# Godotcoffee/AlignGraph2

Measured on AMD Instinct MI355X. Metric: aligned-read-bases/sec through PAGraph build+traverse, higher is better.
Workload: dtype u32

## Files before the change

### aligngraph2_amd/csrc/hip/k1_extract.hip

```cpp
#include "pag_device.hpp"

namespace pagdev {

constexpr int TILE = 1024;
constexpr int CHUNK = 1024;

template <int MAXS>
struct WaveLds {
    uint32_t kept[64];
    uint32_t rank[64];
    uint32_t scode[MAXS];
    uint32_t scnt[MAXS];
    uint32_t srun[MAXS];
    uint32_t st[MAXS];
};
constexpr int MAXS_SPACED = 352;

__device__ __forceinline__ uint32_t load_cols16(const uint32_t *__restrict__ diff, uint64_t diff_off, uint32_t n_cols,
                                                bool back, uint32_t j0, uint32_t *n_lane) {
    if (j0 >= n_cols) {
        *n_lane = 0;
        return 0;
    }
    uint32_t n = n_cols - j0;
    if (n > 16) n = 16;
    *n_lane = n;
    if (!back) return diff[diff_off + (j0 >> 4)];
    int64_t s_lo = (int64_t)n_cols - 16 - (int64_t)j0;
    uint32_t w32;
    if (s_lo >= 0) {
        uint64_t w = diff_off + ((uint64_t)s_lo >> 4);
        uint32_t sh = ((uint32_t)s_lo & 15u) * 2u;
        uint32_t lo = diff[w];
        w32 = lo >> sh;
        if (sh) w32 |= diff[w + 1] << (32 - sh);
    } else {
        uint32_t m = (uint32_t)(-s_lo);
        w32 = diff[diff_off] << (2 * m);
    }
    return rev2(w32);
}

__device__ __forceinline__ void col_masks(uint32_t bits, uint32_t n_lane, uint32_t *emitb, uint32_t *radvb) {
    uint32_t valid = n_lane >= 16 ? 0x55555555u : (((1u << (2 * n_lane)) - 1u) & 0x55555555u);
    uint32_t qd = bits & 0x55555555u, rd = (bits >> 1) & 0x55555555u;
    *emitb = ~(qd & ~rd) & valid;
    *radvb = ~(rd & ~qd) & valid;
}

__global__ __launch_bounds__(64) void colidx_kernel(const pag_aln *__restrict__ aln, uint64_t n_aln,
                                                    const uint32_t *__restrict__ diff,
                                                    const uint64_t *__restrict__ colidx_off, uint2 *__restrict__ colidx) {
    uint64_t ai = blockIdx.x;
    if (ai >= n_aln) return;
    pag_aln al = aln[ai];
    if (!(al.flags & PAG_ALN_ELIGIBLE) || al.query == PAG_NONE) return;
    bool back = (al.flags & PAG_ALN_WALK_BACK) != 0;
    uint32_t n_chunks = (al.n_cols + CHUNK - 1) / CHUNK;
    uint32_t e = 0, r = 0;
    uint64_t base = colidx_off[ai];
    for (uint32_t c = 0; c < n_chunks; ++c) {
        if (lane_id() == 0) colidx[base + c] = make_uint2(e, r);
        uint32_t n_lane, eb, rb;
        uint32_t bits = load_cols16(diff, al.diff_off, al.n_cols, back, c * CHUNK + lane_id() * 16, &n_lane);
        col_masks(bits, n_lane, &eb, &rb);
        e += wave_sum(__popc(eb));
        r += wave_sum(__popc(rb));
    }
}

int launch_colidx(const pag_aln *aln, uint64_t n_aln, const uint32_t *diff, const uint64_t *colidx_off, uint2 *colidx,
                  hipStream_t s) {
    if (n_aln == 0) return PAG_OK;
    colidx_kernel<<<dim3((unsigned)n_aln), dim3(64), 0, s>>>(aln, n_aln, diff, colidx_off, colidx);
    PAG_HIP_TRY(hipGetLastError());
    return PAG_OK;
}

template <typename F>
__device__ __forceinline__ void walk_alignment(const pag_aln &al, const uint32_t *__restrict__ diff,
                                               const uint2 *__restrict__ cidx, uint32_t lo, uint32_t hi, F f) {
    uint32_t q_end = al.q_start + al.n_valid;
    uint32_t a = lo > al.q_start ? lo : al.q_start;
    uint32_t b = hi < q_end ? hi : q_end;
    if (a >= b) return;
    uint32_t e0 = a - al.q_start, e1 = b - al.q_start;
    bool back = (al.flags & PAG_ALN_WALK_BACK) != 0;
    uint32_t n_chunks = (al.n_cols + CHUNK - 1) / CHUNK;
    uint32_t c_lo = 0, c_hi = n_chunks;
    while (c_hi - c_lo > 1) {
        uint32_t mid = (c_lo + c_hi) >> 1;
        if (cidx[mid].x <= e0) c_lo = mid;
        else c_hi = mid;
    }
    for (uint32_t c = c_lo; c < n_chunks; ++c) {
        uint2 pre = cidx[c];
        if (pre.x >= e1) break;
        uint32_t n_lane, eb, rb;
        uint32_t bits = load_cols16(diff, al.diff_off, al.n_cols, back, c * CHUNK + lane_id() * 16, &n_lane);
        col_masks(bits, n_lane, &eb, &rb);
        uint32_t tot;
        uint32_t eex = wave_excl_sum(__popc(eb), &tot) + pre.x;
        uint32_t rex = wave_excl_sum(__popc(rb), &tot) + pre.y;
        uint32_t m = eb;
        while (m) {
            uint32_t bit = __ffs(m) - 1;
            m &= m - 1;
            uint32_t below = (1u << bit) - 1u;
            uint32_t ord = eex + __popc(eb & below);
            if (ord >= e0 && ord < e1) f(al.q_start + ord, al.t_start + rex + __popc(rb & below));
        }
    }
}

__device__ __forceinline__ uint32_t even_bits16(uint32_t x) {
    x &= 0x55555555u;
    x = (x | (x >> 1)) & 0x33333333u;
    x = (x | (x >> 2)) & 0x0F0F0F0Fu;
    x = (x | (x >> 4)) & 0x00FF00FFu;
    return (x | (x >> 8)) & 0xFFFFu;
}
__device__ __forceinline__ uint32_t nth_set_bit16(uint32_t x, uint32_t n) {
    uint32_t pos = 0, c = __popc(x & 0xFFu);
    if (n >= c) n -= c, pos = 8u, x >>= 8;
    c = __popc(x & 0xFu);
    if (n >= c) n -= c, pos += 4u, x >>= 4;
    c = __popc(x & 0x3u);
    if (n >= c) n -= c, pos += 2u, x >>= 2;
    return pos + (n >= (x & 1u) ? 1u : 0u);
}
template <typename G>
__device__ __forceinline__ void walk_kept(const pag_aln &al, const uint32_t *__restrict__ diff, const uint2 *__restrict__ cidx, uint32_t lo,
                                          uint32_t hi, const uint32_t (&kept)[64], const uint32_t (&rank)[64], G g) {
    const uint32_t q_end = al.q_start + al.n_valid;
    const uint32_t a = lo > al.q_start ? lo : al.q_start;
    const uint32_t b = hi < q_end ? hi : q_end;
    if (a >= b) return;
    const uint32_t e0 = a - al.q_start, e1 = b - al.q_start;
    const bool back = (al.flags & PAG_ALN_WALK_BACK) != 0;
    const uint32_t n_chunks = (al.n_cols + CHUNK - 1) / CHUNK;
    uint32_t c_lo = 0, c_hi = n_chunks;
    while (c_hi - c_lo > 1) {
        const uint32_t mid = (c_lo + c_hi) >> 1;
        if (cidx[mid].x <= e0) c_lo = mid;
        else c_hi = mid;
    }
    for (uint32_t c = c_lo; c < n_chunks; ++c) {
        const uint2 pre = cidx[c];
        if (pre.x >= e1) break;
        uint32_t n_lane, eb, rb;
        const uint32_t bits = load_cols16(diff, al.diff_off, al.n_cols, back, c * CHUNK + lane_id() * 16, &n_lane);
        col_masks(bits, n_lane, &eb, &rb);
        const uint32_t ne = __popc(eb);
        uint32_t tot;
        const uint32_t eex = wave_excl_sum(ne, &tot) + pre.x;
        const uint32_t rex = wave_excl_sum(__popc(rb), &tot) + pre.y;
        const uint32_t o_lo = eex > e0 ? eex : e0, o_hi = eex + ne < e1 ? eex + ne : e1;
        if (o_lo >= o_hi) continue;
        const uint32_t d_lo = al.q_start + o_lo - lo, n = o_hi - o_lo;
        const uint32_t w = d_lo >> 4, sh = d_lo & 15u;
        const bool two = sh + n > 16u;
        const uint32_t k0 = kept[w] & 0xFFFFu, k1 = two ? kept[w + 1] & 0xFFFFu : 0u;
        uint32_t km = ((k0 | (k1 << 16)) >> sh) & ((1u << n) - 1u);
        if (!km) continue;
        const uint32_t e16 = even_bits16(eb), r16 = even_bits16(rb);
        const uint32_t r0 = rank[w], r1 = two ? rank[w + 1] : 0u;
        while (km) {
            const uint32_t i = (uint32_t)__ffs((int)km) - 1u;
            km &= km - 1u;
            const uint32_t col = nth_set_bit16(e16, o_lo + i - eex);
            const uint32_t t = al.t_start + rex + __popc(r16 & ((1u << col) - 1u));
            const uint32_t d = d_lo + i;
            const bool first = (d >> 4) == w;
            g((first ? r0 : r1) + __popc((first ? k0 : k1) & ((1u << (d & 15u)) - 1u)), t);
        }
    }
}

__device__ __forceinline__ void lane_codes(const uint32_t *__restrict__ words, uint32_t strand, uint32_t len, uint32_t k,
                                           uint32_t kmask, uint32_t p0, uint32_t n_mine, uint32_t (&code)[16]) {
    uint64_t W = 0;
    uint32_t sh0 = 0;
    if (n_mine) {
        if (strand == 0) {
            uint32_t w0 = p0 >> 4;
            W = (uint64_t)words[w0] | ((uint64_t)words[w0 + 1] << 32);
        } else {
            int64_t a0 = (int64_t)len - (int64_t)k - (int64_t)p0 - 15;
            uint32_t a1 = a0 > 0 ? (uint32_t)a0 : 0u;
            uint32_t w = a1 >> 4, sh = (a1 & 15u) * 2u;
            uint64_t lo64 = (uint64_t)words[w] | ((uint64_t)words[w + 1] << 32);
            W = lo64 >> sh;
            if (sh) W |= (uint64_t)words[w + 2] << (64 - sh);
            sh0 = (uint32_t)((a0 - (int64_t)a1) * 2);
        }
    }
    if (strand == 0) {
        fwd_codes16(W, k, kmask, code);
        return;
    }
#pragma unroll
    for (int j = 0; j < 16; ++j) {
        const uint32_t shj = (uint32_t)(2 * (15 - j)) + sh0;
        const uint32_t x = (uint32_t)(W >> (shj & 63u)) & kmask;
        code[j] = (~x) & kmask;
    }
}

struct LaneWindow {
    uint64_t x = 0;
    uint32_t s0 = 0;
    __device__ __forceinline__ uint32_t code(uint32_t strand, uint32_t kmask, uint32_t j) const {
        if (strand == 0) return (uint32_t)(x >> (s0 - 2u * j)) & kmask;
        return ~(uint32_t)(x >> ((2u * (15u - j) + s0) & 63u)) & kmask;
    }
};
__device__ __forceinline__ LaneWindow lane_window(const uint32_t *__restrict__ words, uint32_t strand, uint32_t len, uint32_t k, uint32_t p0,
                                                  uint32_t n_mine) {
    LaneWindow L;
    if (!n_mine) return L;
    if (strand == 0) {
        const uint32_t w0 = p0 >> 4;
        const uint32_t lo = words[w0], hi = words[w0 + 1];
        L.x = ((uint64_t)rev2(lo) << 32) | (uint64_t)rev2(hi);
        L.s0 = 2u * (32u - k);
    } else {
        const int64_t a0 = (int64_t)len - (int64_t)k - (int64_t)p0 - 15;
        const uint32_t a1 = a0 > 0 ? (uint32_t)a0 : 0u;
        const uint32_t w = a1 >> 4, sh = (a1 & 15u) * 2u;
        const uint64_t lo64 = (uint64_t)words[w] | ((uint64_t)words[w + 1] << 32);
        L.x = lo64 >> sh;
        if (sh) L.x |= (uint64_t)words[w + 2] << (64 - sh);
        L.s0 = (uint32_t)((a0 - (int64_t)a1) * 2);
    }
    return L;
}

constexpr uint32_t SOLID_SLICES = 8;
__global__ __launch_bounds__(64) void solid_mask_kernel(ExtractArgs A, const pag_aln *__restrict__ aln2,
                                                        const uint64_t *__restrict__ qoff2, uint16_t *__restrict__ mask) {
    const uint32_t job = blockIdx.x / SOLID_SLICES, slice = blockIdx.x % SOLID_SLICES;
    const uint32_t lane = lane_id();
    const uint32_t r = A.emit_order[job >> 1];
    const uint32_t strand = job & 1u;
    const uint32_t len = A.read_len[r];
    const uint32_t k = A.k;
    if (len < k) return;
    const uint32_t kmask = k >= 16 ? 0xFFFFFFFFu : ((1u << (2 * k)) - 1u);
    const uint32_t slice_shift = 2 * k - 3;
    const uint32_t *__restrict__ words = (const uint32_t *)(A.packed + A.read_off[r]);
    const uint32_t n_pos = len - k + 1;
    uint32_t lo = 0xFFFFFFFFu, hi = 0;
    for (int db = 0; db < 2; ++db) {
        const pag_aln *al = db == 0 ? A.aln : aln2;
        const uint64_t *qo = db == 0 ? A.query_off : qoff2;
        for (uint64_t ai = qo[r]; ai < qo[r + 1]; ++ai) {
            pag_aln a = al[ai];
            if (!(a.flags & PAG_ALN_ELIGIBLE) || a.q_start == PAG_NONE || a.n_valid == 0) continue;
            if (((a.flags & PAG_ALN_REV_STRAND) ? 1u : 0u) != strand) continue;
            lo = a.q_start < lo ? a.q_start : lo;
            hi = a.q_start + a.n_valid > hi ? a.q_start + a.n_valid : hi;
        }
    }
    if (hi > n_pos) hi = n_pos;
    if (lo >= hi) return;
    uint16_t *m = mask + (uint64_t)slice * A.solid_mask_stride + 2ull * (A.read_off[r] >> 2) + strand;
    for (uint32_t t0 = lo & ~(uint32_t)(TILE - 1); t0 < hi; t0 += TILE) {
        const uint32_t p0 = t0 + lane * 16;
        const uint32_t n_mine = p0 >= n_pos ? 0u : (n_pos - p0 > 16 ? 16u : n_pos - p0);
        if (p0 + 16 <= lo || p0 >= hi || n_mine == 0) continue;
        uint32_t code[16];
        lane_codes(words, strand, len, k, kmask, p0, n_mine, code);
        uint32_t bits = 0;
#pragma unroll
        for (int j = 0; j < 16; ++j)
            if ((uint32_t)j < n_mine && (code[j] >> slice_shift) == slice) bits |= ((A.solid_bits[code[j] >> 5] >> (code[j] & 31u)) & 1u) << j;
        m[2ull * (p0 >> 4)] = (uint16_t)bits;
    }
}

int launch_solid_mask(const ExtractArgs &a, const pag_aln *aln2, const uint64_t *qoff2, uint16_t *mask, hipStream_t s) {
    if (a.n_reads == 0) return PAG_OK;
    solid_mask_kernel<<<dim3(SOLID_SLICES * 2u * a.n_reads), dim3(64), 0, s>>>(a, aln2, qoff2, mask);
    PAG_HIP_TRY(hipGetLastError());
    return PAG_OK;
}
uint32_t solid_mask_slices() { return SOLID_SLICES; }

__device__ __forceinline__ uint32_t tab_get(uint32_t tab, uint32_t s) { return (tab >> (4 * s)) & 15u; }
__device__ __forceinline__ uint32_t byte_compose(uint32_t first, uint32_t then) { return __builtin_amdgcn_perm(then, then, first); }
__device__ __forceinline__ uint32_t byte_get(uint32_t tab, uint32_t s) { return (tab >> (8 * s)) & 255u; }
__device__ __forceinline__ uint32_t tab_compose(uint32_t first, uint32_t then, uint32_t S) {
    uint32_t out = 0;
    for (uint32_t s = 0; s <= S; ++s) out |= tab_get(then, tab_get(first, s)) << (4 * s);
    return out;
}

template <bool EMIT, int MAXS>
__global__ __launch_bounds__(64) void extract_kernel(ExtractArgs A) {
    __shared__ WaveLds<MAXS> L;
    const uint32_t job = A.exec_perm ? A.exec_perm[blockIdx.x] : blockIdx.x;
    const uint32_t lane = lane_id();
    const uint32_t r = A.emit_order[job >> 1];
    const uint32_t strand = job & 1u;
    const uint32_t len = A.read_len[r];
    const uint32_t k = A.k;
    const uint32_t S = A.outer;
    const uint64_t a_lo = A.query_off[r], a_hi = A.query_off[r + 1];
    const uint32_t kmask = k >= 16 ? 0xFFFFFFFFu : ((1u << (2 * k)) - 1u);
    const uint32_t *__restrict__ words = (const uint32_t *)(A.packed + A.read_off[r]);

    auto for_active = [&](auto body) {
        int done = 0;
        for (uint64_t ai = a_lo; ai < a_hi; ++ai) {
            if (A.topk >= 0 && done >= A.topk) break;
            pag_aln al = A.aln[ai];
            if (!(al.flags & PAG_ALN_ELIGIBLE)) continue;
            if (A.cov_ok && !A.cov_ok[ai]) continue;
            ++done;
            if (((al.flags & PAG_ALN_REV_STRAND) ? 1u : 0u) != strand) continue;
            if (al.q_start == PAG_NONE || al.n_valid == 0) continue;
            body(al, ai);
        }
    };

    uint32_t job_samples = 0;
    uint64_t job_tuples = 0;
    bool any = false;
    if (len >= k) for_active([&](const pag_aln &, uint64_t) { any = true; });
    if (!any) {
        if (!EMIT && lane == 0) {
            A.job_samples[A.job_base + job] = 0;
            A.job_tuples[A.job_base + job] = 0;
        }
        return;
    }
    const uint32_t n_pos = len - k + 1;
    bool fast_counts = false;
    if (EMIT) {
        uint32_t n_act = 0;
        bool any_multi = false;
        for_active([&](const pag_aln &al, uint64_t) {
            ++n_act;
            any_multi = any_multi || (A.pass == 0 && A.ctgs[al.target].multi != 0);
        });
        fast_counts = !any_multi && n_act <= 15u;
    }
    const uint64_t tuple_base = EMIT ? A.tuple_off[A.job_base + job] : 0;
    const uint64_t edge_base = EMIT ? A.edge_off[A.job_base + job] : 0;

    uint32_t state = S;
    uint32_t byte_t0 = 0, byte_t1 = 0;
    for (uint32_t st = 0; st < 4u; ++st) {
        byte_t0 |= (st + 1u > S ? S : st + 1u) << (8u * st);
        byte_t1 |= (st + 1u >= S ? 0u : st + 1u) << (8u * st);
    }
    bool carry_valid = false;
    uint32_t carry_pos = 0, carry_code = 0;

    for (uint32_t t0 = 0; t0 < n_pos; t0 += TILE) {
        const uint32_t p0 = t0 + lane * 16;
        const uint32_t t_hi = t0 + TILE < n_pos ? t0 + TILE : n_pos;

        uint32_t ne = 0;
        for_active([&](const pag_aln &al, uint64_t) {
            uint32_t lo = al.q_start > p0 ? al.q_start : p0;
            uint32_t hi = al.q_start + al.n_valid;
            if (hi > p0 + 16) hi = p0 + 16;
            if (hi > n_pos) hi = n_pos;
            if (lo < hi) ne |= ((1u << (hi - p0)) - 1u) & ~((1u << (lo - p0)) - 1u);
        });
        if (__ballot(ne != 0) == 0ull) {
            state = S;
            continue;
        }

        uint32_t cand = 0;
        const uint32_t n_mine = p0 >= n_pos ? 0u : (n_pos - p0 > 16 ? 16u : n_pos - p0);
        LaneWindow win;
        if (EMIT) win = lane_window(words, strand, len, k, p0, n_mine);
        if (A.all_solid) {
            cand = ne;
        } else if (ne) {
            const uint64_t mi = 2ull * ((A.read_off[r] >> 2) + (p0 >> 4)) + strand;
            uint32_t sm = 0;
#pragma unroll
            for (uint32_t sl = 0; sl < SOLID_SLICES; ++sl) sm |= A.solid_mask[(uint64_t)sl * A.solid_mask_stride + mi];
            cand = ne & sm;
        }

        uint32_t v;
        if (S <= 3u) {
            uint32_t tab = 0x03020100u;
#pragma unroll
            for (uint32_t j = 0; j < 16u; ++j)
                if (j < n_mine) tab = byte_compose(tab, ((cand >> j) & 1u) ? byte_t1 : byte_t0);
            uint32_t incl = tab;
#pragma unroll
            for (int d = 1; d < 64; d <<= 1) {
                const uint32_t prev = __shfl_up(incl, d, 64);
                if ((int)lane >= d) incl = byte_compose(prev, incl);
            }
            const uint32_t excl = __shfl_up(incl, 1, 64);
            v = lane == 0 ? state : byte_get(excl, state);
            state = byte_get(__shfl(incl, 63, 64), state);
        } else {
            uint32_t tab = 0;
            for (uint32_t s = 0; s <= S; ++s) tab |= s << (4 * s);
            for (uint32_t j = 0; j < n_mine; ++j) {
                uint32_t c = (cand >> j) & 1u, nt = 0;
                for (uint32_t s = 0; s <= S; ++s) {
                    uint32_t x = tab_get(tab, s);
                    x = (c && x + 1 >= S) ? 0u : (x + 1 > S ? S : x + 1);
                    nt |= x << (4 * s);
                }
                tab = nt;
            }
            uint32_t incl = tab;
#pragma unroll
            for (int d = 1; d < 64; d <<= 1) {
                uint32_t prev = __shfl_up(incl, d, 64);
                if ((int)lane >= d) incl = tab_compose(prev, incl, S);
            }
            uint32_t excl = __shfl_up(incl, 1, 64);
            v = lane == 0 ? state : tab_get(excl, state);
            state = tab_get(__shfl(incl, 63, 64), state);
        }
        uint32_t kept = 0;
        for (uint32_t j = 0; j < n_mine; ++j) {
            uint32_t c = (cand >> j) & 1u;
            if (c && v + 1 >= S) {
                kept |= 1u << j;
                v = 0;
            } else {
                v = v + 1 > S ? S : v + 1;
            }
        }

        uint32_t tile_samples;
        const uint32_t rank0 = wave_excl_sum(__popc(kept), &tile_samples);
        if (tile_samples == 0) continue;

        if (EMIT) {
            uint64_t cnt4 = 0;
            if (fast_counts && kept)
                for_active([&](const pag_aln &al, uint64_t) {
                    uint32_t lo = al.q_start > p0 ? al.q_start : p0;
                    uint32_t hi = al.q_start + al.n_valid;
                    if (hi > p0 + 16) hi = p0 + 16;
                    if (lo >= hi) return;
                    uint32_t m = kept & ((1u << (hi - p0)) - 1u) & ~((1u << (lo - p0)) - 1u);
                    while (m) {
                        cnt4 += 1ull << (4u * (uint32_t)(__ffs(m) - 1));
                        m &= m - 1u;
                    }
                });
            __syncthreads();
            L.kept[lane] = kept;
            L.rank[lane] = rank0;
            uint32_t last_pos = 0, last_code = 0;
            if (kept) {
                const uint32_t jl = 31u - (uint32_t)__clz((int)kept);
                last_pos = p0 + jl;
                last_code = win.code(strand, kmask, jl);
            }
            uint64_t has = __ballot(kept != 0);
            uint64_t before = has & lanemask_lt();
            int src = before ? 63 - __clzll((long long)before) : 0;
            uint32_t pp = __shfl(last_pos, src, 64), pc = __shfl(last_code, src, 64);
            bool pvalid = before != 0;
            if (!pvalid) {
                pp = carry_pos;
                pc = carry_code;
                pvalid = carry_valid;
            }
            uint32_t i = 0;
            for (uint32_t m = kept; m; m &= m - 1u) {
                const uint32_t j = (uint32_t)__ffs((int)m) - 1u;
                const uint32_t cj = win.code(strand, kmask, j);
                const uint32_t s_local = rank0 + i;
                L.scode[s_local] = cj;
                L.scnt[s_local] = (uint32_t)(cnt4 >> (4 * j)) & 15u;
                L.srun[s_local] = 0;
                if (pvalid) {
                    const uint64_t slot = edge_base + (uint64_t)job_samples + s_local - 1;
                    A.ekey[slot] = pc;
                    A.eval[slot] = ((uint64_t)cj << 32) | ((uint64_t)(p0 + j - pp) << 1) | (uint64_t)A.pass;
                }
                pp = p0 + j;
                pc = cj;
                pvalid = true;
                ++i;
            }
            int top = 63 - __clzll((long long)has);
            carry_pos = __shfl(last_pos, top, 64);
            carry_code = __shfl(last_code, top, 64);
            carry_valid = true;
            __syncthreads();
        }

        uint32_t tile_tuples = 0;
        if (!EMIT) {
            for_active([&](const pag_aln &al, uint64_t ai) {
                bool multi = A.pass == 0 && A.ctgs[al.target].multi != 0;
                if (!multi) {
                    uint32_t lo = al.q_start > p0 ? al.q_start : p0;
                    uint32_t hi = al.q_start + al.n_valid;
                    if (hi > p0 + 16) hi = p0 + 16;
                    if (lo < hi) tile_tuples += __popc(kept & ((1u << (hi - p0)) - 1u) & ~((1u << (lo - p0)) - 1u));
                } else {
                    __syncthreads();
                    L.kept[lane] = kept;
                    __syncthreads();
                    const pag_ctg cg = A.ctgs[al.target];
                    walk_alignment(al, A.diff, A.colidx + A.colidx_off[ai], t0, t_hi, [&](uint32_t q, uint32_t t) {
                        uint32_t d = q - t0;
                        if ((L.kept[d >> 4] >> (d & 15u)) & 1u)
                            tile_tuples += A.ctg_ent_off[cg.map_off + t + 1] - A.ctg_ent_off[cg.map_off + t];
                    });
                }
            });
            job_tuples += wave_sum(tile_tuples);
        } else {
            if (!fast_counts) for_active([&](const pag_aln &al, uint64_t ai) {
                const bool ctg_pass = A.pass == 0;
                pag_ctg cg{};
                if (ctg_pass) cg = A.ctgs[al.target];
                walk_alignment(al, A.diff, A.colidx + A.colidx_off[ai], t0, t_hi, [&](uint32_t q, uint32_t t) {
                    uint32_t d = q - t0;
                    uint32_t km = L.kept[d >> 4];
                    if ((km >> (d & 15u)) & 1u) {
                        uint32_t s_local = L.rank[d >> 4] + __popc(km & ((1u << (d & 15u)) - 1u));
                        uint32_t c = ctg_pass ? A.ctg_ent_off[cg.map_off + t + 1] - A.ctg_ent_off[cg.map_off + t] : 1u;
                        L.scnt[s_local] += c;
                    }
                });
                __syncthreads();
// ... 138 lines not shown
```

### aligngraph2_amd/csrc/hip/pag_api.hip

```cpp
#include <algorithm>
#include <cstdlib>
#include <cstring>
#include <new>
#include <string>
#include <thread>
#include <chrono>
#include <vector>

#include "pag_device.hpp"
#include "pagraph_debug.h"

using namespace pagdev;

#include "pag_graph_impl.hpp"
#include "walker_grid.hpp"

namespace {

template <typename T>
int stage(const T *src, uint64_t n, bool on_device, DevBuf &own, const T **out, hipStream_t s) {
    if (on_device) {
        *out = src;
        return PAG_OK;
    }
// ... 182 lines not shown
        hipError_t e = hipStreamCreate(&g->stream);
        if (e == hipSuccess) e = hipMalloc((void **)&g->solid_bits, (size_t)words * 4 + 64);
        if (e == hipSuccess)
            e = hipMemcpy(g->solid_bits, bits, (size_t)words * 4, bits_on_device ? hipMemcpyDeviceToDevice : hipMemcpyHostToDevice);
        if (e != hipSuccess) {
            set_error("pag_create_from_bitmap: %s", hipGetErrorString(e));
            rc = PAG_EFAULT;
        }
    }
    if (rc != PAG_OK && g) {
        pag_destroy(g);
        g = nullptr;
    }
    if (err) *err = rc;
    return g;
}

void pag_destroy(pag_graph *g) {
    if (!g) return;
    hipSetDevice(g->device);
    free_graph_results(g);
    drain_deferred(g);
    for (auto &sl : g->pool) slot_free(g, sl);
    for (auto &sl : g->cpool) slot_free(g, sl);
    if (g->deliver_stream) hipStreamDestroy(g->deliver_stream);
    for (OwnedBuf *b : {&g->wq_host, &g->wq_next, &g->path_store, &g->pin_host, &g->walk_arena, &g->dump_tables, &g->dump_scratch}) b->release();
    for (OwnedBuf &c : g->fetch_chunks) c.release();
    g->fetch_chunks.clear();
    for (hipStream_t ws : g->walk_streams) hipStreamDestroy(ws);
    if (g->solid_bits) hipFree(g->solid_bits);
    if (g->stream) hipStreamDestroy(g->stream);
    delete g;
}

uint64_t pag_solid_count(const pag_graph *g) { return g ? g->n_solid : 0; }

int pag_reset(pag_graph *g) {
    if (!g) return PAG_EINVAL;
    hipSetDevice(g->device);
    free_graph_results(g);
    g->stats = pag_build_stats{};
    return PAG_OK;
}

}

namespace {

struct Extracted {
    uint64_t T = 0, E = 0, T1 = 0, E1 = 0;
};

struct StreamBufs {
    DevBuf tk0, tv0, tk1, tv1, ek0, ev0, ek1, ev1, sorttmp;
    explicit StreamBufs(pag_graph *g)
        : tk0(g, ps::TK0), tv0(g, ps::TV0), tk1(g, ps::TK1), tv1(g, ps::TV1), ek0(g, ps::EK0), ev0(g, ps::EV0), ek1(g, ps::EK1), ev1(g, ps::EV1),
          sorttmp(g, ps::SORT_TMP) {}
    int alloc(uint64_t T, uint64_t E) {
        int rc;
        if ((rc = tk0.alloc((T + 1) * 4)) || (rc = tv0.alloc((T + 1) * 8)) || (rc = ek0.alloc((E + 1) * 4)) || (rc = ev0.alloc((E + 1) * 8)) ||
            (rc = tk1.alloc((T + 1) * 4)) || (rc = tv1.alloc((T + 1) * 12)) || (rc = ek1.alloc((E + 1) * 4)) || (rc = ev1.alloc((E + 1) * 12)))
            return rc;
        return sorttmp.alloc(sort_tmp_bytes(std::max(T, E)));
    }
};

int extract_stage(pag_graph *g, const pag_build_input *in, uint64_t emit_lo, uint64_t emit_hi, Extracted *out, hipEvent_t ev_begin,
                  hipEvent_t ev_end) {
    hipStream_t s = g->stream;
    const bool dev = in->on_device != 0;
    const uint32_t n_reads_all = (uint32_t)in->reads.n_seqs;
    const uint32_t n_reads = (uint32_t)(emit_hi - emit_lo);
    const uint64_t n_jobs = 4ull * n_reads;
    int rc;
    if (ev_begin) PAG_HIP_TRY(hipEventRecord(ev_begin, s));

    DevBuf b_roff(g, ps::IN_ROFF), b_rlen(g, ps::IN_RLEN), b_packed(g, ps::IN_PACKED), b_order(g, ps::IN_ORDER), b_aln1(g, ps::IN_ALN1), b_q1(g, ps::IN_Q1),
        b_d1(g, ps::IN_D1), b_aln2(g, ps::IN_ALN2), b_q2(g, ps::IN_Q2), b_d2(g, ps::IN_D2), b_ctg(g, ps::IN_CTG), b_eoff(g, ps::IN_EOFF), b_ent(g, ps::IN_ENT),
        b_ref(g, ps::IN_REF);
    const uint64_t *d_roff;
    const uint32_t *d_rlen, *d_order, *d_d1, *d_d2, *d_eoff, *d_ent;
    const uint8_t *d_packed;
    const pag_aln *d_aln1, *d_aln2;
    const uint64_t *d_q1, *d_q2;
    const pag_ctg *d_ctg;
    const pag_ref *d_ref;
    if ((rc = stage(in->reads.byte_off, n_reads_all, dev, b_roff, &d_roff, s))) return rc;
    if ((rc = stage(in->reads.len, n_reads_all, dev, b_rlen, &d_rlen, s))) return rc;
    if ((rc = stage(in->reads.packed, in->reads.packed_bytes, dev, b_packed, &d_packed, s))) return rc;
    if ((rc = stage(in->emit_order, n_reads_all, dev, b_order, &d_order, s))) return rc;
    if ((rc = stage(in->read_to_ctg.aln, in->read_to_ctg.n_aln, dev, b_aln1, &d_aln1, s))) return rc;
    if ((rc = stage(in->read_to_ctg.query_off, (uint64_t)n_reads_all + 1, dev, b_q1, &d_q1, s))) return rc;
    if ((rc = stage(in->read_to_ctg.diff, in->read_to_ctg.n_diff_words, dev, b_d1, &d_d1, s))) return rc;
    if ((rc = stage(in->read_to_ref.aln, in->read_to_ref.n_aln, dev, b_aln2, &d_aln2, s))) return rc;
    if ((rc = stage(in->read_to_ref.query_off, (uint64_t)n_reads_all + 1, dev, b_q2, &d_q2, s))) return rc;
    if ((rc = stage(in->read_to_ref.diff, in->read_to_ref.n_diff_words, dev, b_d2, &d_d2, s))) return rc;
    if ((rc = stage(in->ctgs, in->n_ctgs, dev, b_ctg, &d_ctg, s))) return rc;
    if ((rc = stage(in->ctg_ent_off, in->n_ctg_ent_off, dev, b_eoff, &d_eoff, s))) return rc;
    if ((rc = stage(in->ctg_ent, in->n_ctg_ent, dev, b_ent, &d_ent, s))) return rc;
    if ((rc = stage(in->refs, in->n_refs, dev, b_ref, &d_ref, s))) return rc;
    d_order += emit_lo;

    std::vector<pag_ref> refs_host((size_t)in->n_refs);
    if (in->n_refs) {
        if (dev) PAG_HIP_TRY(hipMemcpy(refs_host.data(), in->refs, in->n_refs * sizeof(pag_ref), hipMemcpyDeviceToHost));
        else std::memcpy(refs_host.data(), in->refs, in->n_refs * sizeof(pag_ref));
    }

    const uint64_t n_aln1 = in->read_to_ctg.n_aln, n_aln2 = in->read_to_ref.n_aln;
    DevBuf b_covok(g, ps::COV_OK), b_covtmp(g, ps::COV_TMP);
    if ((rc = b_covok.alloc(n_aln2 + 16))) return rc;
    size_t cov_bytes = cov_tmp_bytes(refs_host.data(), in->n_refs);
    if ((rc = b_covtmp.alloc(cov_bytes))) return rc;
    if ((rc = launch_cov_filter(d_aln2, n_aln2, d_ref, refs_host.data(), in->n_refs, in->cov_filter,
                                b_covok.as<uint8_t>(), b_covtmp.p, cov_bytes, s)))
        return rc;

    DevBuf b_cc(g, ps::CI_CC), b_cio1(g, ps::CI_OFF1), b_cio2(g, ps::CI_OFF2), b_ci1(g, ps::CI_1), b_ci2(g, ps::CI_2), b_scan(g, ps::X_SCAN), b_tot(g, ps::X_TOT);
    uint64_t n_alnmax = std::max(n_aln1, n_aln2);
    if ((rc = b_cc.alloc((n_alnmax + 1) * 4))) return rc;
    if ((rc = b_cio1.alloc((n_aln1 + 1) * 8))) return rc;
    if ((rc = b_cio2.alloc((n_aln2 + 1) * 8))) return rc;
    if ((rc = b_scan.alloc(scan_tmp_bytes(std::max<uint64_t>(n_alnmax, n_jobs) + 1)))) return rc;
    if ((rc = b_tot.alloc(64))) return rc;
    uint64_t *d_tot = b_tot.as<uint64_t>();
    uint64_t n_ci[2] = {0, 0};
    for (int pass = 0; pass < 2; ++pass) {
        const pag_aln *al = pass == 0 ? d_aln1 : d_aln2;
        uint64_t na = pass == 0 ? n_aln1 : n_aln2;
        DevBuf &off = pass == 0 ? b_cio1 : b_cio2;
        if (na) {
            chunk_counts<<<dim3((unsigned)((na + 255) / 256)), dim3(256), 0, s>>>(al, na, b_cc.as<uint32_t>());
            if ((rc = scan_u32_to_u64(b_cc.as<uint32_t>(), off.as<uint64_t>(), na, d_tot + pass, b_scan.p, s))) return rc;
            PAG_HIP_TRY(hipMemcpyAsync(&n_ci[pass], d_tot + pass, 8, hipMemcpyDeviceToHost, s));
        }
    }
    PAG_HIP_TRY(hipStreamSynchronize(s));
    for (int pass = 0; pass < 2; ++pass) {
        const pag_aln *al = pass == 0 ? d_aln1 : d_aln2;
        uint64_t na = pass == 0 ? n_aln1 : n_aln2;
        DevBuf &off = pass == 0 ? b_cio1 : b_cio2;
        DevBuf &ci = pass == 0 ? b_ci1 : b_ci2;
        if ((rc = ci.alloc((n_ci[pass] + 1) * sizeof(uint2)))) return rc;
        if ((rc = launch_colidx(al, na, pass == 0 ? d_d1 : d_d2, off.as<uint64_t>(), ci.as<uint2>(), s))) return rc;
    }

    DevBuf b_js(g, ps::K1_JS), b_jt(g, ps::K1_JT), b_je(g, ps::K1_JE), b_toff(g, ps::K1_TOFF), b_eoff2(g, ps::K1_EOFF);
    if ((rc = b_js.alloc((n_jobs + 1) * 4))) return rc;
    if ((rc = b_jt.alloc((n_jobs + 1) * 4))) return rc;
    if ((rc = b_je.alloc((n_jobs + 1) * 4))) return rc;
    if ((rc = b_toff.alloc((n_jobs + 1) * 8))) return rc;
    if ((rc = b_eoff2.alloc((n_jobs + 1) * 8))) return rc;
    DevBuf b_smask(g, ps::SOLID_MASK);
    if (!g->all_solid) {
        if ((rc = b_smask.alloc((in->reads.packed_bytes / 4 + 16) * 2 * sizeof(uint16_t) * solid_mask_slices()))) return rc;
    }
    ExtractArgs xa[2];
    for (int pass = 0; pass < 2; ++pass) {
        ExtractArgs &a = xa[pass];
        a = ExtractArgs{};
        a.read_off = d_roff;
        a.read_len = d_rlen;
        a.packed = d_packed;
        a.emit_order = d_order;
        a.n_reads = n_reads;
        a.aln = pass == 0 ? d_aln1 : d_aln2;
        a.query_off = pass == 0 ? d_q1 : d_q2;
        a.diff = pass == 0 ? d_d1 : d_d2;
        a.colidx_off = (pass == 0 ? b_cio1 : b_cio2).as<uint64_t>();
        a.colidx = (pass == 0 ? b_ci1 : b_ci2).as<uint2>();
        a.cov_ok = pass == 0 ? nullptr : b_covok.as<uint8_t>();
        a.pass = pass;
        a.topk = pass == 0 ? in->topk_ctg : in->topk_ref;
        a.ctgs = d_ctg;
        a.ctg_ent_off = d_eoff;
        a.ctg_ent = d_ent;
        a.refs = d_ref;
        a.solid_bits = g->solid_bits;
        a.solid_mask = g->all_solid ? nullptr : b_smask.as<uint16_t>();
        a.solid_mask_stride = (in->reads.packed_bytes / 4 + 16) * 2;
        a.all_solid = g->all_solid;
        a.k = g->k;
        a.outer = in->outer_sample;
        a.job_samples = b_js.as<uint32_t>();
        a.job_tuples = b_jt.as<uint32_t>();
        a.job_base = (uint32_t)(pass * 2ull * n_reads);
    }
    DevBuf b_pk0(g, ps::K1_PK0), b_pv0(g, ps::K1_PV0), b_pk1(g, ps::K1_PK1), b_pv1(g, ps::K1_PV1), b_ptmp(g, ps::K1_PTMP), b_perm(g, ps::K1_PERM);
    {
        const uint64_t nj0 = 2ull * n_reads;
        if (nj0 >= 4096) {
            if ((rc = b_pk0.alloc(nj0 * 4)) || (rc = b_pv0.alloc(nj0 * 8)) || (rc = b_pk1.alloc(nj0 * 4)) || (rc = b_pv1.alloc(nj0 * 8)) ||
                (rc = b_ptmp.alloc(sort_tmp_bytes(nj0))) || (rc = b_perm.alloc(nj0 * 4)))
                return rc;
            if ((rc = launch_exec_perm(xa[0], b_pk0.as<uint32_t>(), b_pv0.as<uint64_t>(), b_pk1.as<uint32_t>(), b_pv1.as<uint64_t>(), b_ptmp.p,
                                       b_perm.as<uint32_t>(), s)))
                return rc;
            xa[0].exec_perm = b_perm.as<uint32_t>();
        }
    }
    if (!g->all_solid && (rc = launch_solid_mask(xa[0], d_aln2, d_q2, b_smask.as<uint16_t>(), s))) return rc;
    for (int pass = 0; pass < 2; ++pass)
        if ((rc = launch_extract(xa[pass], false, s))) return rc;
    uint64_t T = 0, E = 0, T1 = 0, E1 = 0;
    if (n_jobs) {
        edge_counts<<<dim3((unsigned)((n_jobs + 255) / 256)), dim3(256), 0, s>>>(b_js.as<uint32_t>(), n_jobs,
                                                                                 b_je.as<uint32_t>());
        if ((rc = scan_u32_to_u64(b_jt.as<uint32_t>(), b_toff.as<uint64_t>(), n_jobs, d_tot + 2, b_scan.p, s))) return rc;
        if ((rc = scan_u32_to_u64(b_je.as<uint32_t>(), b_eoff2.as<uint64_t>(), n_jobs, d_tot + 3, b_scan.p, s))) return rc;
        PAG_HIP_TRY(hipMemcpyAsync(&T, d_tot + 2, 8, hipMemcpyDeviceToHost, s));
        PAG_HIP_TRY(hipMemcpyAsync(&E, d_tot + 3, 8, hipMemcpyDeviceToHost, s));
        PAG_HIP_TRY(hipMemcpyAsync(&T1, b_toff.as<uint64_t>() + 2ull * n_reads, 8, hipMemcpyDeviceToHost, s));
        PAG_HIP_TRY(hipMemcpyAsync(&E1, b_eoff2.as<uint64_t>() + 2ull * n_reads, 8, hipMemcpyDeviceToHost, s));
        PAG_HIP_TRY(hipStreamSynchronize(s));
    }

    DevBuf b_tk0(g, ps::TK0), b_tv0(g, ps::TV0), b_ek0(g, ps::EK0), b_ev0(g, ps::EV0);
    if ((rc = b_tk0.alloc((T + 1) * 4)) || (rc = b_tv0.alloc((T + 1) * 8)) || (rc = b_ek0.alloc((E + 1) * 4)) || (rc = b_ev0.alloc((E + 1) * 8))) return rc;
    for (int pass = 0; pass < 2; ++pass) {
        ExtractArgs &a = xa[pass];
        a.tuple_off = b_toff.as<uint64_t>();
        a.edge_off = b_eoff2.as<uint64_t>();
        a.tkey = b_tk0.as<uint32_t>();
        a.tval = b_tv0.as<uint64_t>();
        a.ekey = b_ek0.as<uint32_t>();
        a.eval = b_ev0.as<uint64_t>();
        if ((rc = launch_extract(a, true, s))) return rc;
    }
    if (ev_end) PAG_HIP_TRY(hipEventRecord(ev_end, s));
    out->T = T;
    out->E = E;
    out->T1 = T1;
    out->E1 = E1;
    return PAG_OK;
}

int build_stage(pag_graph *g, uint32_t eps, const Extracted &x, pag_build_stats *st_out, hipEvent_t *ev ) {
    hipStream_t s = g->stream;
    const uint64_t T = x.T, E = x.E, T1 = x.T1, E1 = x.E1;
    int rc;
    StreamBufs sb(g);
    if ((rc = sb.alloc(T, E))) return rc;
    PAG_HIP_TRY(hipEventRecord(ev[0], s));

    int t_in0 = 1, e_in0 = 1, passes = 0;
    float ms_scatter_t = 0.f, ms_scatter_e = 0.f;
    if ((rc = sort_pairs(sb.tk0.as<uint32_t>(), sb.tv0.as<uint64_t>(), sb.tk1.as<uint32_t>(), sb.tv1.as<uint64_t>(), T,
                         2 * (int)g->k, sb.sorttmp.p, &t_in0, s, &ms_scatter_t, &passes)))
        return rc;
    if ((rc = sort_pairs(sb.ek0.as<uint32_t>(), sb.ev0.as<uint64_t>(), sb.ek1.as<uint32_t>(), sb.ev1.as<uint64_t>(), E,
                         2 * (int)g->k, sb.sorttmp.p, &e_in0, s, &ms_scatter_e, nullptr)))
        return rc;
    PAG_HIP_TRY(hipEventRecord(ev[1], s));
    DevBuf *tk = t_in0 ? &sb.tk0 : &sb.tk1, *tv = t_in0 ? &sb.tv0 : &sb.tv1;
    DevBuf *ek = e_in0 ? &sb.ek0 : &sb.ek1, *evb = e_in0 ? &sb.ev0 : &sb.ev1;
    DevBuf b_tscr(g, ps::T_SCR), b_escr(g, ps::E_SCR);
    uint64_t *t_scratch, *e_scratch;
    if (t_in0) {
        t_scratch = sb.tv1.as<uint64_t>();
    } else {
        if ((rc = b_tscr.alloc((T + 1) * 12))) return rc;
        t_scratch = b_tscr.as<uint64_t>();
    }
    if (e_in0) {
        e_scratch = sb.ev1.as<uint64_t>();
    } else {
        if ((rc = b_escr.alloc((E + 1) * 12))) return rc;
        e_scratch = b_escr.as<uint64_t>();
    }

    DevBuf b_tseg(g, ps::T_SEG), b_tcnt(g, ps::T_CNT), b_eseg(g, ps::E_SEG), b_long(g, ps::SEG_LONG), b_lcnt(g, ps::SEG_LCNT), b_ctr(g, ps::CTR);
    if ((rc = b_tseg.alloc((T + 1) * 4))) return rc;
    if ((rc = b_tcnt.alloc((T + 1) * 2))) return rc;
    if ((rc = b_eseg.alloc((E + 1) * 4))) return rc;
    if ((rc = b_long.alloc((std::max(T, E) / 32 + 2) * 8))) return rc;
    if ((rc = b_lcnt.alloc(64))) return rc;
    if ((rc = b_ctr.alloc(128))) return rc;
    uint64_t *ctr_dev = b_ctr.as<uint64_t>();
    ClusterOut co{b_tseg.as<uint32_t>(), b_tcnt.as<uint16_t>(), ctr_dev};
    const bool wide = g->n_solid != 0 && T > 10 * g->n_solid;
    if ((rc = launch_cluster(tk->as<uint32_t>(), tv->as<uint64_t>(), t_scratch, T, eps, co, b_long.as<uint64_t>(),
                             b_lcnt.as<uint32_t>(), s, wide)))
        return rc;
    PAG_HIP_TRY(hipEventRecord(ev[2], s));
    EdgeOut eo{b_eseg.as<uint32_t>(), ctr_dev + 4};
    if ((rc = launch_edges(ek->as<uint32_t>(), evb->as<uint64_t>(), e_scratch, E, eo, b_long.as<uint64_t>(),
                           b_lcnt.as<uint32_t>(), s, wide)))
        return rc;
    uint64_t ctr[8] = {0, 0, 0, 0, 0, 0, 0, 0};
    PAG_HIP_TRY(hipMemcpyAsync(ctr, b_ctr.p, 64, hipMemcpyDeviceToHost, s));
    PAG_HIP_TRY(hipEventRecord(ev[3], s));
    PAG_HIP_TRY(hipStreamSynchronize(s));

    pag_build_stats st{};
    const uint64_t T2 = T - T1, E2 = E - E1;
    const uint64_t L_ctg = ctr[0], L_all = ctr[1], U_all = ctr[4], U_1 = ctr[5];
    st.n_tuples[0] = T1;
    st.n_tuples[1] = T2;
    st.n_edges[0] = E1;
    st.n_edges[1] = E2;
    st.merge_edge[0] = E1 - U_1;
    st.total_pos[0] = T1;
    st.merge_pos[0] = T1 - L_ctg;
    st.merge_edge[1] = U_1 + E2 - U_all;
    st.total_pos[1] = L_ctg + T2;
    st.merge_pos[1] = L_ctg + T2 - L_all;
    st.n_nodes = ctr[2];
    st.n_pos = L_all;
    st.n_uniq_edges = U_all;
    float ms = 0.f;
    hipEventElapsedTime(&ms, ev[0], ev[1]);
    st.ms_sort = ms;
    hipEventElapsedTime(&ms, ev[1], ev[2]);
    st.ms_cluster = ms;
    hipEventElapsedTime(&ms, ev[2], ev[3]);
    st.ms_edges = ms;
    st.ms_sort_kernel = ms_scatter_t;
    st.sort_records = T;
    (void)passes;
    (void)ms_scatter_e;

    g->n_t = T;
    g->n_e = E;
    g->tkey = tk->as<uint32_t>();
    g->tval = tv->as<uint64_t>();
    g->tseg = b_tseg.as<uint32_t>();
    g->tcnt = b_tcnt.as<uint16_t>();
    g->ekey = ek->as<uint32_t>();
    g->eval = evb->as<uint64_t>();
    g->eseg = b_eseg.as<uint32_t>();
    g->stats = st;
    *st_out = st;
    return PAG_OK;
// ... 494 lines not shown
```

Before: 4.076 billion.

## Filter solid-mask k-mers by slice bitwise and compact lookups to members

The solid-mask kernel now computes, with bitwise ops on the packed window, which of a lane's 16 k-mers fall into the block's slice, and looks up solid_bits only for those members, two per wave-level iteration. Before, it computed all 16 codes and did a predicated gather for each. The strand branch is specialised at compile time, and the mask layout changes from strand-interleaved to strand-planar, which makes mask writes and reads contiguous per strand. The cost is a ballot-driven loop with extra divergence, plus a layout change that must match the consumer indexing.

```diff
diff --git a/aligngraph2_amd/csrc/hip/k1_extract.hip b/aligngraph2_amd/csrc/hip/k1_extract.hip
--- a/aligngraph2_amd/csrc/hip/k1_extract.hip
+++ b/aligngraph2_amd/csrc/hip/k1_extract.hip
@@ -1,4 +1,7 @@
+#include <type_traits>
+
 #include "pag_device.hpp"
+#include "lane_window.hpp"
 
 namespace pagdev {
 
@@ -113,13 +116,6 @@
     }
 }
 
-__device__ __forceinline__ uint32_t even_bits16(uint32_t x) {
-    x &= 0x55555555u;
-    x = (x | (x >> 1)) & 0x33333333u;
-    x = (x | (x >> 2)) & 0x0F0F0F0Fu;
-    x = (x | (x >> 4)) & 0x00FF00FFu;
-    return (x | (x >> 8)) & 0xFFFFu;
-}
 __device__ __forceinline__ uint32_t nth_set_bit16(uint32_t x, uint32_t n) {
     uint32_t pos = 0, c = __popc(x & 0xFFu);
     if (n >= c) n -= c, pos = 8u, x >>= 8;
@@ -177,64 +173,6 @@
     }
 }
 
-__device__ __forceinline__ void lane_codes(const uint32_t *__restrict__ words, uint32_t strand, uint32_t len, uint32_t k,
-                                           uint32_t kmask, uint32_t p0, uint32_t n_mine, uint32_t (&code)[16]) {
-    uint64_t W = 0;
-    uint32_t sh0 = 0;
-    if (n_mine) {
-        if (strand == 0) {
-            uint32_t w0 = p0 >> 4;
-            W = (uint64_t)words[w0] | ((uint64_t)words[w0 + 1] << 32);
-        } else {
-            int64_t a0 = (int64_t)len - (int64_t)k - (int64_t)p0 - 15;
-            uint32_t a1 = a0 > 0 ? (uint32_t)a0 : 0u;
-            uint32_t w = a1 >> 4, sh = (a1 & 15u) * 2u;
-            uint64_t lo64 = (uint64_t)words[w] | ((uint64_t)words[w + 1] << 32);
-            W = lo64 >> sh;
-            if (sh) W |= (uint64_t)words[w + 2] << (64 - sh);
-            sh0 = (uint32_t)((a0 - (int64_t)a1) * 2);
-        }
-    }
-    if (strand == 0) {
-        fwd_codes16(W, k, kmask, code);
-        return;
-    }
-#pragma unroll
-    for (int j = 0; j < 16; ++j) {
-        const uint32_t shj = (uint32_t)(2 * (15 - j)) + sh0;
-        const uint32_t x = (uint32_t)(W >> (shj & 63u)) & kmask;
-        code[j] = (~x) & kmask;
-    }
-}
-
-struct LaneWindow {
-    uint64_t x = 0;
-    uint32_t s0 = 0;
-    __device__ __forceinline__ uint32_t code(uint32_t strand, uint32_t kmask, uint32_t j) const {
-        if (strand == 0) return (uint32_t)(x >> (s0 - 2u * j)) & kmask;
-        return ~(uint32_t)(x >> ((2u * (15u - j) + s0) & 63u)) & kmask;
-    }
-};
-__device__ __forceinline__ LaneWindow lane_window(const uint32_t *__restrict__ words, uint32_t strand, uint32_t len, uint32_t k, uint32_t p0,
-                                                  uint32_t n_mine) {
-    LaneWindow L;
-    if (!n_mine) return L;
-    if (strand == 0) {
-        const uint32_t w0 = p0 >> 4;
-        const uint32_t lo = words[w0], hi = words[w0 + 1];
-        L.x = ((uint64_t)rev2(lo) << 32) | (uint64_t)rev2(hi);
-        L.s0 = 2u * (32u - k);
-    } else {
-        const int64_t a0 = (int64_t)len - (int64_t)k - (int64_t)p0 - 15;
-        const uint32_t a1 = a0 > 0 ? (uint32_t)a0 : 0u;
-        const uint32_t w = a1 >> 4, sh = (a1 & 15u) * 2u;
-        const uint64_t lo64 = (uint64_t)words[w] | ((uint64_t)words[w + 1] << 32);
-        L.x = lo64 >> sh;
-        if (sh) L.x |= (uint64_t)words[w + 2] << (64 - sh);
-        L.s0 = (uint32_t)((a0 - (int64_t)a1) * 2);
-    }
-    return L;
-}
 
 constexpr uint32_t SOLID_SLICES = 8;
 __global__ __launch_bounds__(64) void solid_mask_kernel(ExtractArgs A, const pag_aln *__restrict__ aln2,
@@ -247,7 +185,6 @@
     const uint32_t k = A.k;
     if (len < k) return;
     const uint32_t kmask = k >= 16 ? 0xFFFFFFFFu : ((1u << (2 * k)) - 1u);
-    const uint32_t slice_shift = 2 * k - 3;
     const uint32_t *__restrict__ words = (const uint32_t *)(A.packed + A.read_off[r]);
     const uint32_t n_pos = len - k + 1;
     uint32_t lo = 0xFFFFFFFFu, hi = 0;
@@ -264,19 +201,38 @@
     }
     if (hi > n_pos) hi = n_pos;
     if (lo >= hi) return;
-    uint16_t *m = mask + (uint64_t)slice * A.solid_mask_stride + 2ull * (A.read_off[r] >> 2) + strand;
-    for (uint32_t t0 = lo & ~(uint32_t)(TILE - 1); t0 < hi; t0 += TILE) {
-        const uint32_t p0 = t0 + lane * 16;
-        const uint32_t n_mine = p0 >= n_pos ? 0u : (n_pos - p0 > 16 ? 16u : n_pos - p0);
-        if (p0 + 16 <= lo || p0 >= hi || n_mine == 0) continue;
-        uint32_t code[16];
-        lane_codes(words, strand, len, k, kmask, p0, n_mine, code);
-        uint32_t bits = 0;
-#pragma unroll
-        for (int j = 0; j < 16; ++j)
-            if ((uint32_t)j < n_mine && (code[j] >> slice_shift) == slice) bits |= ((A.solid_bits[code[j] >> 5] >> (code[j] & 31u)) & 1u) << j;
-        m[2ull * (p0 >> 4)] = (uint16_t)bits;
-    }
+    uint16_t *m = mask + (uint64_t)slice * A.solid_mask_stride + (uint64_t)strand * (A.solid_mask_stride >> 1) + (A.read_off[r] >> 2);
+    auto tiles = [&](auto strand_c) {
+        constexpr uint32_t STRAND = decltype(strand_c)::value;
+        for (uint32_t t0 = lo & ~(uint32_t)(TILE - 1); t0 < hi; t0 += TILE) {
+            const uint32_t p0 = t0 + lane * 16;
+            const uint32_t n_pos_mine = p0 >= n_pos ? 0u : (n_pos - p0 > 16 ? 16u : n_pos - p0);
+            const bool visit = !(p0 + 16 <= lo || p0 >= hi || n_pos_mine == 0);
+            const uint32_t n_mine = visit ? n_pos_mine : 0u;
+            const LaneWindow win = lane_window(words, STRAND, len, k, p0, n_mine);
+            uint32_t mem = slice_members(win.x, STRAND, k, win.s0, n_mine, slice);
+            uint32_t bits = 0;
+            while (__ballot(mem != 0u) != 0ull) {
+                uint32_t w0 = 0, w1 = 0, c0 = 0, c1 = 0, j0 = 0, j1 = 0;
+                if (mem) {
+                    j0 = (uint32_t)__ffs((int)mem) - 1u;
+                    mem &= mem - 1u;
+                    c0 = win.code(STRAND, kmask, j0);
+                    w0 = A.solid_bits[c0 >> 5];
+                }
+                if (mem) {
+                    j1 = (uint32_t)__ffs((int)mem) - 1u;
+                    mem &= mem - 1u;
+                    c1 = win.code(STRAND, kmask, j1);
+                    w1 = A.solid_bits[c1 >> 5];
+                }
+                bits |= (((w0 >> (c0 & 31u)) & 1u) << j0) | (((w1 >> (c1 & 31u)) & 1u) << j1);
+            }
+            if (visit) m[p0 >> 4] = (uint16_t)bits;
+        }
+    };
+    if (strand == 0) tiles(std::integral_constant<uint32_t, 0u>{});
+    else tiles(std::integral_constant<uint32_t, 1u>{});
 }
 
 int launch_solid_mask(const ExtractArgs &a, const pag_aln *aln2, const uint64_t *qoff2, uint16_t *mask, hipStream_t s) {
@@ -382,7 +338,7 @@
         if (A.all_solid) {
             cand = ne;
         } else if (ne) {
-            const uint64_t mi = 2ull * ((A.read_off[r] >> 2) + (p0 >> 4)) + strand;
+            const uint64_t mi = (uint64_t)strand * (A.solid_mask_stride >> 1) + (A.read_off[r] >> 2) + (p0 >> 4);
             uint32_t sm = 0;
 #pragma unroll
             for (uint32_t sl = 0; sl < SOLID_SLICES; ++sl) sm |= A.solid_mask[(uint64_t)sl * A.solid_mask_stride + mi];
diff --git a/aligngraph2_amd/csrc/hip/lane_window.hpp b/aligngraph2_amd/csrc/hip/lane_window.hpp
--- /dev/null
+++ b/aligngraph2_amd/csrc/hip/lane_window.hpp
@@ -0,0 +1,79 @@
+#pragma once
+#include <stdint.h>
+
+#if defined(__HIPCC__)
+#define PAG_LW_HD __host__ __device__ inline
+#else
+#define PAG_LW_HD inline
+#endif
+
+namespace pagdev {
+
+PAG_LW_HD uint32_t brev32(uint32_t x) {
+#if defined(__HIP_DEVICE_COMPILE__)
+    return __brev(x);
+#else
+    x = (x >> 16) | (x << 16);
+    x = ((x & 0xFF00FF00u) >> 8) | ((x & 0x00FF00FFu) << 8);
+    x = ((x & 0xF0F0F0F0u) >> 4) | ((x & 0x0F0F0F0Fu) << 4);
+    x = ((x & 0xCCCCCCCCu) >> 2) | ((x & 0x33333333u) << 2);
+    return ((x & 0xAAAAAAAAu) >> 1) | ((x & 0x55555555u) << 1);
+#endif
+}
+PAG_LW_HD uint32_t rev2_groups(uint32_t x) {
+    x = brev32(x);
+    return ((x & 0xAAAAAAAAu) >> 1) | ((x & 0x55555555u) << 1);
+}
+PAG_LW_HD uint32_t even_bits16(uint32_t x) {
+    x &= 0x55555555u;
+    x = (x | (x >> 1)) & 0x33333333u;
+    x = (x | (x >> 2)) & 0x0F0F0F0Fu;
+    x = (x | (x >> 4)) & 0x00FF00FFu;
+    return (x | (x >> 8)) & 0xFFFFu;
+}
+
+struct LaneWindow {
+    uint64_t x = 0;
+    uint32_t s0 = 0;
+    PAG_LW_HD uint32_t code(uint32_t strand, uint32_t kmask, uint32_t j) const {
+        if (strand == 0) return (uint32_t)(x >> (s0 - 2u * j)) & kmask;
+        return ~(uint32_t)(x >> ((2u * (15u - j) + s0) & 63u)) & kmask;
+    }
+};
+PAG_LW_HD LaneWindow lane_window(const uint32_t *__restrict__ words, uint32_t strand, uint32_t len, uint32_t k, uint32_t p0, uint32_t n_mine) {
+    LaneWindow L;
+    if (!n_mine) return L;
+    if (strand == 0) {
+        const uint32_t w0 = p0 >> 4;
+        const uint32_t lo = words[w0], hi = words[w0 + 1];
+        L.x = ((uint64_t)rev2_groups(lo) << 32) | (uint64_t)rev2_groups(hi);
+        L.s0 = 2u * (32u - k);
+    } else {
+        const int64_t a0 = (int64_t)len - (int64_t)k - (int64_t)p0 - 15;
+        const uint32_t a1 = a0 > 0 ? (uint32_t)a0 : 0u;
+        const uint32_t w = a1 >> 4, sh = (a1 & 15u) * 2u;
+        const uint64_t lo64 = (uint64_t)words[w] | ((uint64_t)words[w + 1] << 32);
+        L.x = lo64 >> sh;
+        if (sh) L.x |= (uint64_t)words[w + 2] << (64 - sh);
+        L.s0 = (uint32_t)((a0 - (int64_t)a1) * 2);
+    }
+    return L;
+}
+
+PAG_LW_HD uint32_t slice_members(uint64_t x, uint32_t strand, uint32_t k, uint32_t s0, uint32_t n_mine, uint32_t slice) {
+    uint64_t y;
+    if (strand == 0) {
+        y = x >> 30;
+    } else {
+        const int32_t sh = (int32_t)s0 + 2 * (int32_t)k - 4;
+        y = ~(sh >= 0 ? x >> sh : x << -sh);
+    }
+    const uint64_t qa = ((slice & 1u) ? 0ull : 0xAAAAAAAAAAAAAAAAull) | ((slice & 2u) ? 0ull : 0x5555555555555555ull);
+    const uint64_t qb = (slice & 4u) ? 0ull : 0xAAAAAAAAAAAAAAAAull;
+    const uint64_t a = y ^ qa;
+    const uint64_t b = y ^ qb;
+    const uint32_t m = (uint32_t)a & (uint32_t)(a >> 1) & (uint32_t)(b >> 2) & 0xAAAAAAAAu;
+    return even_bits16(brev32(m)) & ((1u << n_mine) - 1u);
+}
+
+}
diff --git a/aligngraph2_amd/csrc/hip/pag_api.hip b/aligngraph2_amd/csrc/hip/pag_api.hip
--- a/aligngraph2_amd/csrc/hip/pag_api.hip
+++ b/aligngraph2_amd/csrc/hip/pag_api.hip
@@ -358,8 +358,9 @@
     if ((rc = b_toff.alloc((n_jobs + 1) * 8))) return rc;
     if ((rc = b_eoff2.alloc((n_jobs + 1) * 8))) return rc;
     DevBuf b_smask(g, ps::SOLID_MASK);
+    const uint64_t solid_mask_half = in->reads.packed_bytes / 4 + 16;
     if (!g->all_solid) {
-        if ((rc = b_smask.alloc((in->reads.packed_bytes / 4 + 16) * 2 * sizeof(uint16_t) * solid_mask_slices()))) return rc;
+        if ((rc = b_smask.alloc(solid_mask_half * 2 * sizeof(uint16_t) * solid_mask_slices()))) return rc;
     }
     ExtractArgs xa[2];
     for (int pass = 0; pass < 2; ++pass) {
@@ -384,7 +385,7 @@
         a.refs = d_ref;
         a.solid_bits = g->solid_bits;
         a.solid_mask = g->all_solid ? nullptr : b_smask.as<uint16_t>();
-        a.solid_mask_stride = (in->reads.packed_bytes / 4 + 16) * 2;
+        a.solid_mask_stride = solid_mask_half * 2;
         a.all_solid = g->all_solid;
         a.k = g->k;
         a.outer = in->outer_sample;
```

Result: no change. 4.050 billion (-0.7%).
